# liangheming/simple_pose

Measured on AMD Instinct MI355X. Metric: images/sec fwd+decode, ResNet50-DConv 256x192 bs=128, higher is better.
Workload: dtype f32; 1 GPU; ResNet50-DConv 256x192 bs=128 per GPU, fp32 forward (NCHW in -> heat maps) + GaussTaylor decode, eval-mode BN, conditioned random weights; images_per_gpu=128, global_batch=128, parallelism=replicas x1 (no collective), ranks=1 process(es), one per GPU, launch=stream launches, tile_table=profiles/r06_dconv_f32_tiles.json, batches_in_flight=2, decode=in line, HSA_ENABLE_IPC_MODE_LEGACY=0

## Files before the change

include/simple_pose_hip.h:

```cpp
#ifndef SIMPLE_POSE_HIP_H
#define SIMPLE_POSE_HIP_H

#include <stdint.h>

#ifdef __cplusplus
extern "C" {
#endif

#define SP_OK 0
#define SP_EINVAL (-1)
#define SP_ELAUNCH (-2)

#define SP_ABI_VERSION 36

#define SP_CONV_RELU 0x1u
#define SP_CONV_OUT_NCHW 0x2u
#define SP_CONV_PIXEL_SHUFFLE 0x4u
#define SP_CONV_OUT_F32 0x10u
#define SP_CONV_BN_Y_MASK 0x20u
#define SP_CONV_BF16 0x8u
#define SP_CONV_HARDSWISH 0x40u
#define SP_CONV_OUT_SLICE 0x80u

typedef struct sp_conv_desc {
// ... 44 lines not shown
int sp_basic_block_c64(const sp_conv_desc* desc, const void* x, const void* w1_packed, const float* scale1, const float* shift1,
                       const void* w2_packed, const float* scale2, const float* shift2, void* y, void* stream);

int sp_dual_pw_bf16_ok(int64_t rows, int c_main, int c_short, int c_out);
int sp_dual_pw_f32_ok(int64_t rows, int c_main, int c_short, int c_out);
int sp_dual_pw_f32(const float* a_main, const float* w_main_packed, const float* scale_main, const float* shift_main, const float* a_short,
                   const float* w_short_packed, const float* scale_short, const float* shift_short, float* y, int64_t rows, int c_main, int c_short,
                   int c_out, int relu, void* stream);
int sp_dual_pw_bf16(const void* a_main, const void* w_main_packed, const float* scale_main, const float* shift_main, const void* a_short,
                    const void* w_short_packed, const float* scale_short, const float* shift_short, void* y, int64_t rows, int c_main, int c_short,
                    int c_out, int relu, void* stream);
int sp_pw_chain_f32_ok(int64_t rows, int c_mid, int c_out, int c_next);
int sp_pw_chain_f32(const float* t, const float* w3_packed, const float* scale3, const float* shift3, const float* residual, float* y,
                    const float* w1_packed, const float* scale1, const float* shift1, float* t_next, int64_t rows, int c_mid, int c_out, int c_next,
                    void* stream);
int sp_bottleneck_c64_ok(const sp_conv_desc* desc);
int sp_bottleneck_c64(const sp_conv_desc* desc, const void* x, const void* w1_packed, const float* scale1, const float* shift1,
                      const void* w2_packed, const float* scale2, const float* shift2, const void* w3_packed, const float* scale3,
                      const float* shift3, void* y, void* stream);

int sp_stem7_pool_ok(int batch, int h, int w);
int sp_stem7_pool(const float* x, const void* w_packed, int k_pad, const float* scale, const float* shift, void* y, int bf16,
                  int batch, int h, int w, void* stream);
int sp_stem7_pool_u8(const unsigned char* crops_bgr, const float* mean_rgb_host, const void* w_packed, int k_pad, const float* scale,
                     const float* shift, void* y, int bf16, int batch, int h, int w, void* stream);

int sp_hrnet_transition1_ok(int c_in, int h, int w);
int sp_hrnet_transition1(const void* x, int batch, int h, int w, const void* wa_packed, int k_pad, const float* scale_a, const float* shift_a,
                         const void* wb_packed, const float* scale_b, const float* shift_b, void* y_hi, void* y_lo, void* stream);
int sp_hrnet_stem_ok(int batch, int h, int w);
// ... 339 lines not shown
```

simple_pose_amd/_lib.py:

```python
from __future__ import annotations

import ctypes
import os
from ctypes import c_double, c_float, c_int, c_int32, c_int64, c_uint32, c_void_p

from .build import LIB_PATH as _DEFAULT_LIB_PATH

LIB_PATH = os.environ.get("SIMPLE_POSE_HIP_LIB", _DEFAULT_LIB_PATH)

SP_CONV_RELU = 0x1
SP_CONV_OUT_NCHW = 0x2
SP_CONV_PIXEL_SHUFFLE = 0x4
SP_CONV_BF16 = 0x8
SP_CONV_OUT_F32 = 0x10
SP_CONV_BN_Y_MASK = 0x20
SP_CONV_HARDSWISH = 0x40
SP_CONV_OUT_SLICE = 0x80
SP_LETTERBOX_FOCUS, SP_LETTERBOX_U8 = 0, 1
SP_YOLO_NMS_MAX_CANDIDATES, SP_YOLO_NMS_MAX_DET = 32768, 1024
SP_COCO_MAX_JOINTS, SP_COCO_MAX_GT_PER_IMAGE, SP_COCO_MAX_DT_PER_IMAGE, SP_COCO_MAX_DETS = 64, 128, 2048, 32
SP_COCO_DT_XY_F64, SP_COCO_DT_SCORE_F64, SP_COCO_GT_CROWD, SP_COCO_GT_IGNORE = 1, 2, 1, 2
CONV_TILES =((128, 128), (64, 128), (128, 64), (64, 64), (256, 64), (128, 32))
ABI_VERSION = 36
SP_CONV_KERNEL_IGEMM, SP_CONV_KERNEL_RING, SP_CONV_KERNEL_PW, SP_CONV_KERNEL_RING_LW, SP_CONV_KERNEL_RING_LW4 = 0, 1, 2, 3, 4
RING_LW4_TILES = ((192, 128), (128, 128), (96, 128), (256, 128), (128, 256), (96, 256), (64, 128))
RING_LW_TILES = ((256, 128), (128, 256), (256, 64), (128, 128), (192, 128))
RING_TILES = ((256, 256), (256, 128), (128, 256), (256, 64), (128, 128), (192, 128), (192, 256))


class HipLibraryError(RuntimeError):
    pass


class ConvDesc(ctypes.Structure):
    _fields_ = [(n, c_int32) for n in (
        "batch", "in_h", "in_w", "c_in", "grid_h", "grid_w", "c_out", "n_pad", "taps_h", "taps_w", "k_pad", "stride",
        "dy0", "dy_step", "dx0", "dx_step", "out_h", "out_w", "out_c", "oy_mul", "oy_add", "ox_mul", "ox_add",
# ... 122 lines not shown
    "sp_bn_fold_bwd_apply_nhwc": (c_int, [_P, c_int, _P, _P, _P, _P, _P, c_int, c_int, _P, _P, _P, c_int64, c_int64, c_int, _P, _P, _P, _P, _P, _P, c_int, _P]),
    "sp_bn_bwd_sums_from_conv": (c_int, [_P, _P, c_int, c_int, c_int, _P, _P, _P]),
    "sp_bn_bwd_sums_from_conv_pair": (c_int, [_P, _P, _P, c_int, c_int, c_int, _P, _P, _P, _P, _P]),
    "sp_u8hwc_bgr_to_nhwc": (c_int, [_P, _P, c_int, c_int, c_int, c_int, _P, _P]),
    "sp_nchw_to_nhwc4_bf16": (c_int, [_P, _P, c_int, c_int, c_int, c_int, _P]),
    "sp_conv3x3_direct_ok": (c_int, [ctypes.POINTER(ConvDesc)]),
    "sp_conv3x3_direct": (c_int, [ctypes.POINTER(ConvDesc), _P, _P, _P, _P, _P, _P, _P]),
    "sp_basic_block_c32_ok": (c_int, [ctypes.POINTER(ConvDesc)]),
    "sp_basic_block_c32": (c_int, [ctypes.POINTER(ConvDesc), _P, _P, _P, _P, _P, _P, _P, _P, _P]),
    "sp_basic_block_c64_ok": (c_int, [ctypes.POINTER(ConvDesc)]),
    "sp_basic_block_c64": (c_int, [ctypes.POINTER(ConvDesc), _P, _P, _P, _P, _P, _P, _P, _P, _P]),
    "sp_dual_pw_bf16_ok": (c_int, [c_int64, c_int, c_int, c_int]),
    "sp_dual_pw_f32_ok": (c_int, [c_int64, c_int, c_int, c_int]),
    "sp_dual_pw_f32": (c_int, [_P, _P, _P, _P, _P, _P, _P, _P, _P, c_int64, c_int, c_int, c_int, c_int, _P]),
    "sp_dual_pw_bf16": (c_int, [_P, _P, _P, _P, _P, _P, _P, _P, _P, c_int64, c_int, c_int, c_int, c_int, _P]),
    "sp_pw_chain_f32_ok": (c_int, [c_int64, c_int, c_int, c_int]),
    "sp_pw_chain_f32": (c_int, [_P, _P, _P, _P, _P, _P, _P, _P, _P, _P, c_int64, c_int, c_int, c_int, _P]),
    "sp_bottleneck_c64_ok": (c_int, [ctypes.POINTER(ConvDesc)]),
    "sp_conv2d_pw_ok": (c_int, [ctypes.POINTER(ConvDesc)]),
    "sp_hrnet_stem_ok": (c_int, [c_int, c_int, c_int]),
    "sp_hrnet_stem": (c_int, [_P, _P, c_int, _P, _P, _P, _P, _P, _P, c_int, c_int, c_int, _P]),
    "sp_hrnet_transition1_ok": (c_int, [c_int, c_int, c_int]),
    "sp_hrnet_transition1": (c_int, [_P, c_int, c_int, c_int, _P, c_int, _P, _P, _P, _P, _P, _P, _P, _P]),
    "sp_stem7_pool_ok": (c_int, [c_int, c_int, c_int]),
    "sp_stem7_pool": (c_int, [_P, _P, c_int, _P, _P, _P, c_int, c_int, c_int, c_int, _P]),
    "sp_stem7_pool_u8": (c_int, [_P, ctypes.POINTER(ctypes.c_float), _P, c_int, _P, _P, _P, c_int, c_int, c_int, c_int, _P]),
    "sp_bottleneck_c64": (c_int, [ctypes.POINTER(ConvDesc), _P, _P, _P, _P, _P, _P, _P, _P, _P, _P, _P, _P]),
    "sp_masked_mse": (c_int, [_P, _P, _P, c_int, c_int, c_int, _P, _P, _P, _P]),
    "sp_conv_packed_dims": (c_int, [c_int, c_int, c_int, ctypes.POINTER(c_int), ctypes.POINTER(c_int)]),
    "sp_pack_conv_weights": (c_int, [_P, c_int, c_int, c_int, c_int, c_int, c_int, c_int, c_int, c_int, c_int, _P, c_int, _P]),
# ... 41 lines not shown
        for name, (res, args) in SYMBOLS.items():
            fn = getattr(handle, name)
            fn.restype, fn.argtypes = res, args
        if handle.sp_abi_version() != ABI_VERSION:
            raise HipLibraryError(f"ABI mismatch: library {handle.sp_abi_version()} vs binding {ABI_VERSION}")
        _lib = handle
    return _lib


def conv_kernel_name(desc, has_residual: bool = False, variant: int = 0) -> str:
    buf = ctypes.create_string_buffer(256)
    check(lib().sp_conv2d_kernel_name(desc, int(has_residual), variant, buf, 256), "sp_conv2d_kernel_name")
    return buf.value.decode()


def check(rc: int, what: str = ""):
    if rc != 0:
        msg = lib().sp_last_error().decode("utf-8", "replace")
        raise HipLibraryError(f"{what or 'libsimple_pose_hip'} failed (code {rc}): {msg}")


def ptr(t):
    return None if t is None else t.data_ptr()


import threading

_pin = threading.local()


# ... 51 lines not shown
```

simple_pose_amd/csrc/conv_igemm.hip:

```cpp
#include "sp_common.h"
#include <stdlib.h>
#include <type_traits>

#ifdef SP_DIAG
__device__ unsigned long long sp_dbg[4096 * 4 * 12];
extern "C" int sp_debug_read(unsigned long long* dst, int n) {
    return (int)hipMemcpyFromSymbol(dst, HIP_SYMBOL(sp_dbg), sizeof(unsigned long long) * n, 0, hipMemcpyDeviceToHost);
}
extern "C" int sp_debug_clear() {
    static unsigned long long z[4096 * 4 * 12];
    return (int)hipMemcpyToSymbol(HIP_SYMBOL(sp_dbg), z, sizeof(z), 0, hipMemcpyHostToDevice);
}
#define SP_STAMP_ALWAYS(var)                                                                \
    unsigned long long var;                                                                 \
    __builtin_amdgcn_sched_barrier(0);                                                      \
    asm volatile("s_memtime %0\n\ts_waitcnt lgkmcnt(0)" : "=s"(var)::"memory");           \
    __builtin_amdgcn_sched_barrier(0);
#ifdef SP_DIAG_LIGHT
#define SP_STAMP(var) unsigned long long var = 0;
#else
#define SP_STAMP(var) SP_STAMP_ALWAYS(var)
#endif
#else
#define SP_STAMP(var)
// ... 906 lines not shown
        if ((a.flags & SP_CONV_BF16) && !(a.flags & SP_CONV_OUT_F32)) return launch_t<BM, BN, WR, WC, true, true, false, false, true>(a, phases, uniform, stream);
        if (a.flags & SP_CONV_BF16) return launch_t<BM, BN, WR, WC, true, false, false, false, true>(a, phases, uniform, stream);
        return launch_t<BM, BN, WR, WC, false, false, false, false, true>(a, phases, uniform, stream);
    }
    if (a.stats_s) {
        if (a.flags & SP_CONV_BF16) return launch_t<BM, BN, WR, WC, true, true, true>(a, phases, uniform, stream);
        return launch_t<BM, BN, WR, WC, false, false, true>(a, phases, uniform, stream);
    }
    if (a.flags & SP_CONV_BF16) {
        if (a.flags & SP_CONV_OUT_F32) return launch_t<BM, BN, WR, WC, true, false, false>(a, phases, uniform, stream);
        return launch_t<BM, BN, WR, WC, true, true, false>(a, phases, uniform, stream);
    }
    return launch_t<BM, BN, WR, WC, false, false, false>(a, phases, uniform, stream);
}

}

extern "C" int sp_conv2d_default_tile(const sp_conv_desc* d, int* tile_m, int* tile_n);
int sp_conv_ring_launch(const sp_conv_desc* d, const void* x, const void* w_packed, const float* scale, const float* shift,
                        const void* residual, void* y, void* stream);
int sp_conv_pw_launch(const sp_conv_desc* d, const void* x, const void* w_packed, const float* scale, const float* shift,
                      const void* residual, void* y, void* stream);

static int tile_rows_per_block(int, int) { return 1; }

static int g_tap_skip = -1;
static bool tap_skip_enabled() {
    if (g_tap_skip < 0) { const char* e = getenv("SP_CONV_TAP_SKIP"); g_tap_skip = (e && atoi(e) == 0) ? 0 : 1; }
    return g_tap_skip != 0;
}
// ... 292 lines not shown
        return conv_fwd_impl(&descs[0], dz, w_packed[0], nullptr, nullptr, accumulate, dx, sum_g, sum_g_xhat, stats_rows_capacity, stream, &src, &phs);
    }
    return conv_fwd_impl(&descs[0], dz, w_packed[0], nullptr, nullptr, accumulate, dx, nullptr, nullptr, 0, stream, nullptr, &phs);
}

extern "C" int sp_conv2d_dgrad_bn_bwd_stats_macc(const sp_conv_desc* d, const void* dz, const void* w_packed, const void* acc_dy, const void* acc_mask,
                                                void* dx, const void* bn_y, const void* bn_z, const float* bn_mean, const float* bn_invstd, float* sum_g,
                                                float* sum_g_xhat, const void* bn2_z, const float* bn2_mean, const float* bn2_invstd, float* sum_g_xhat2,
                                                int stats_rows_capacity, void* stream) {
    SP_REQUIRE(acc_dy && acc_mask, "sp_conv2d_dgrad_bn_bwd_stats_macc: null accumulate operand");
    SP_REQUIRE(!bn2_z || (bn2_mean && bn2_invstd && sum_g_xhat2), "sp_conv2d_dgrad_bn_bwd_stats_macc: null pointer");
    BnBwdSrc src = {bn_y, bn_z, bn_mean, bn_invstd, bn2_z, bn2_mean, bn2_invstd, sum_g_xhat2};
    src.res_mask = acc_mask;
    return conv_fwd_impl(d, dz, w_packed, nullptr, nullptr, acc_dy, dx, sum_g, sum_g_xhat, stats_rows_capacity, stream, &src);
}
```

simple_pose_amd/engine.py:

```python
from __future__ import annotations

import ctypes
import os

from dataclasses import dataclass, field
from typing import Dict, List, Optional, Tuple

import torch

from . import _lib, conv_geometry
from ._lib import ConvDesc, SP_CONV_BF16, SP_CONV_HARDSWISH, SP_CONV_OUT_NCHW, SP_CONV_OUT_SLICE, SP_CONV_PIXEL_SHUFFLE, SP_CONV_RELU
from .conv_geometry import n_pad_for, round_up as _round_up

BN_EPS = 1e-5


class HipPacker:

    @staticmethod
    def _dims(c_out: int, k: int, bf16: bool) -> Tuple[int, int]:
        n_pad, k_pad = ctypes.c_int(0), ctypes.c_int(0)
        _lib.check(_lib.lib().sp_conv_packed_dims(c_out, k, int(bf16), ctypes.byref(n_pad), ctypes.byref(k_pad)), "sp_conv_packed_dims")
        return n_pad.value, k_pad.value

# ... 174 lines not shown
                                              P(bufs[op.dst]), stream), op.name)
        elif op.kind == "bneck64":
            op.desc.batch = B
            w1, s1, h1, w3, s3, h3 = op.args
            _lib.check(lib.sp_bottleneck_c64(op.desc, P(bufs[op.src]), P(w1), P(s1), P(h1), P(op.w), P(op.scale), P(op.shift), P(w3), P(s3), P(h3),
                                             P(bufs[op.dst]), stream), op.name)
        elif op.kind == "dual1x1":
            w_s, s_s, h_s, rows_per_image, relu = op.args
            fn = lib.sp_dual_pw_bf16 if op.w.element_size() == 2 else lib.sp_dual_pw_f32
            _lib.check(fn(P(bufs[op.src]), P(op.w), P(op.scale), P(op.shift), P(bufs[op.res]), P(w_s), P(s_s), P(h_s), P(bufs[op.dst]),
                                           B * rows_per_image, 64, 64, 256, relu, stream), op.name)
        elif op.kind == "pwchain":
            w1, s1, h1, rows_per_image, c_next, _ = op.args
            _lib.check(lib.sp_pw_chain_f32(P(bufs[op.src]), P(op.w), P(op.scale), P(op.shift), P(bufs[op.res]), P(bufs[op.dst]), P(w1), P(s1), P(h1),
                                           P(bufs[op.dst2]), B * rows_per_image, 64, 256, c_next, stream), op.name)
        elif op.kind == "stem7":
            h, w, k_pad, unfused = op.args
            src = bufs[op.src]
            if src.dtype == torch.uint8:
                mean = (ctypes.c_float * 3)(0.485, 0.456, 0.406)
                _lib.check(lib.sp_stem7_pool_u8(P(src), mean, P(op.w), k_pad, P(op.scale), P(op.shift), P(bufs[op.dst]), int(self.dtype == "bf16"),
                                                B, h, w, stream), op.name)
            else:
                _lib.check(lib.sp_stem7_pool(P(src), P(op.w), k_pad, P(op.scale), P(op.shift), P(bufs[op.dst]), int(self.dtype == "bf16"),
                                             B, h, w, stream), op.name)
        elif op.kind == "htrans":
            h, w, k_pad, wb, sb, hb, _ = op.args
            _lib.check(lib.sp_hrnet_transition1(P(bufs[op.src]), B, h, w, P(op.w), k_pad, P(op.scale), P(op.shift), P(wb), P(sb), P(hb),
                                                P(bufs[op.dst]), P(bufs[op.dst2]), stream), op.name)
        elif op.kind == "hstem":
# ... 195 lines not shown
                        print(f"  {op.name:28s} {cand[0]:3d}x{cand[1]:<3d} k{cand[2]} {timed[-1][0] * 1e3:8.1f} us")
                timed.sort()
                ranked[key] = timed
                best = timed[0]
                if len(timed) > 1 and timed[1][0] < 1.08 * timed[0][0]:
                    ta, tb = [], []
                    for _ in range(rounds):
                        ta.append(time_once(op, timed[0][1], 3 * reps))
                        tb.append(time_once(op, timed[1][1], 3 * reps))
                    ma, mb = sorted(ta)[rounds // 2], sorted(tb)[rounds // 2]
                    best = (ma, timed[0][1]) if ma <= mb else (mb, timed[1][1])
                chosen[key] = best[1]
            apply(op, chosen[key])
            report[op.name] = chosen[key]
            by_key.setdefault(key, []).append(op)
        self.tuned_for_batch = B
        n_lanes = 1 + max((op.lane for op in self.ops), default=0)
        if refine is None:
            refine = self.multi_stream and n_lanes > 1
        if in_situ and not (self.multi_stream and n_lanes > 1):
            report.update(self._retime_in_situ(x, by_key, ranked, chosen, apply, verbose))
        if refine:
            report.update(self._refine_on_whole_step(x, by_key, ranked, chosen, apply, verbose))
        return report

    def _retime_in_situ(self, x, by_key, ranked, chosen, apply, verbose, top: int = 4, reps: int = 3) -> Dict[str, Tuple[int, int, int]]:
        lib = _lib.lib()
        B = x.shape[0]
        bufs = dict(self._alloc(B, x.device))
        bufs["input"] = x
# ... 60 lines not shown
            for cand in alts:
                for op in by_key[key]:
                    apply(op, cand)
                t = min(self._step_ms(x), self._step_ms(x))
                if t < base * 0.996:
                    if verbose:
                        print(f"  refine {by_key[key][0].name:28s} x{len(by_key[key])}: {chosen[key]} -> {cand}: step {base:.3f} -> {t:.3f} ms")
                    base, chosen[key] = t, cand
                else:
                    for op in by_key[key]:
                        apply(op, chosen[key])
            for op in by_key[key]:
                changed[op.name] = chosen[key]
        return changed

    def tiles(self) -> Dict[str, Tuple[int, int, int]]:
        return {op.name: ((-1, -1, 0) if op.direct else (op.desc.tile_m, op.desc.tile_n, op.desc.kernel)) for op in self.ops if op.kind == "conv"}

    def set_tiles(self, tiles: Dict[str, Tuple[int, ...]], batch: int) -> None:
        for op in self.ops:
            if op.kind == "conv" and op.name in tiles:
                t = [int(v) for v in tiles[op.name]]
                if op.desc.c_in_group:
                    if t[0] > 0 and t[1] == op.desc.c_in_group and (len(t) < 3 or t[2] == _lib.SP_CONV_KERNEL_IGEMM):
                        op.desc.tile_m = t[0]
                    continue
                op.direct = t[0] < 0
                if not op.direct:
                    op.desc.tile_m, op.desc.tile_n = t[0], t[1]
                    op.desc.kernel = t[2] if len(t) > 2 else _lib.SP_CONV_KERNEL_IGEMM
        self.tuned_for_batch = batch

    @property
    def flops_per_image(self) -> int:
        return sum(op.flops for op in self.ops)
# ... 140 lines not shown
                del table[key]
        self._hm = [None] * self.depth


class ProgramBuilder:

    def __init__(self, in_h: int, in_w: int, dtype: str = "fp32", packer=None):
        if dtype not in ("fp32", "bf16"):
            raise ValueError(dtype)
        self.packer = packer or HipPacker()
        self.fuse_blocks = False
        self.fuse_blocks64 = False
        self.fuse_bottlenecks = False
        self.fuse_tail = os.environ.get("SP_FUSE_TAIL", "1") != "0"
        self.fuse_chain = os.environ.get("SP_FUSE_CHAIN", "1") != "0"
        self.fuse_stem = True
        self.fuse_terms = True
        self.fuse_transition = True
        self.p = Program(dtype=dtype)
        self.bf16 = dtype == "bf16"
        self.cpad = 8 if self.bf16 else 4
        self.p.shapes["input"] = (in_h, in_w, 3)
        self._n = 0
        self.lane = 0

    def _add(self, op: Op) -> None:
        op.lane = self.lane
        self.p.ops.append(op)

    def _fresh(self, stem: str) -> str:
# ... 128 lines not shown
    def dual_pointwise_tail(self, main: str, w3, s3, h3, short: str, wd, sd_, hd, name: str) -> Optional[str]:
        h, w, c = self.p.shapes[main]
        hs, ws_, cs = self.p.shapes[short]
        ok = _lib.lib().sp_dual_pw_bf16_ok if self.bf16 else _lib.lib().sp_dual_pw_f32_ok
        if not (self.fuse_tail and (h, w) == (hs, ws_) and c == 64 and cs == 64 and tuple(w3.shape) == (256, 64, 1, 1)
                and tuple(wd.shape) == (256, 64, 1, 1) and ok(h * w, 64, 64, 256)):
            return None
        p3, pd = self.packer.conv(w3, bf16=self.bf16)[0], self.packer.conv(wd, bf16=self.bf16)[0]
        if tuple(p3.shape) != (256, 64) or tuple(pd.shape) != (256, 64):
            return None
        dst = self._fresh(name)
        self.p.shapes[dst] = (h, w, 256)
        self._add(Op("dual1x1", main, dst, res=short, w=p3, scale=s3, shift=h3, args=(pd, sd_, hd, h * w, 1), name=name, flops=2 * h * w * 2 * 64 * 256))
        return dst

    def deconv_k4s2p1(self, src: str, weight: torch.Tensor, *, scale=None, shift=None, relu: bool = False,
                      name: str = "deconv") -> str:
        h, w, c = self.p.shapes[src]
        I, O = weight.shape[:2]
        assert I == c
        packed, n_pad = self.packer.deconv(weight, bf16=self.bf16)
        d = conv_geometry.deconv_k4s2p1_fwd(h, w, I, O, n_pad, (SP_CONV_RELU if relu else 0) | (SP_CONV_BF16 if self.bf16 else 0))
        dst = self._fresh(name)
        self.p.shapes[dst] = (2 * h, 2 * w, O)
        self._add(Op("conv", src, dst, desc=d, w=packed, scale=scale, shift=shift,
                             name=name, flops=2 * h * w * I * O * 16))
        return dst

    def pixel_shuffle(self, src: str) -> str:
        h, w, c = self.p.shapes[src]
# ... 66 lines not shown
        y = b.bottleneck_c64(x, sd[p + ".conv1.weight"], s1, h1, sd[p + ".conv2.weight"], s2, h2, sd[p + ".conv3.weight"], s3, h3, name=p)
        if y is not None:
            return y
    s1, h1 = _bn(b, sd, p + ".bn1")
    t = b.conv(x, sd[p + ".conv1.weight"], scale=s1, shift=h1, relu=True, name=p + ".conv1")
    s2, h2 = _bn(b, sd, p + ".bn2")
    w2 = sd[p + ".conv2.weight"]
    t = b.conv(t, w2, stride=stride, pad=1, scale=s2, shift=h2, relu=True, name=p + ".conv2", groups=w2.shape[0] // w2.shape[1])
    idn = x
    if (p + ".downsample.0.weight") in sd and stride == 1 and (p + ".se.fc.0.weight") not in sd and w2.shape[0] == w2.shape[1]:
        sdn, hdn = _bn(b, sd, p + ".downsample.1")
        s3, h3 = _bn(b, sd, p + ".bn3")
        y = b.dual_pointwise_tail(t, sd[p + ".conv3.weight"], s3, h3, x, sd[p + ".downsample.0.weight"], sdn, hdn, name=p + ".conv3+downsample")
        if y is not None:
            return y
    if (p + ".downsample.0.weight") in sd:
        sdn, hdn = _bn(b, sd, p + ".downsample.1")
        idn = b.conv(x, sd[p + ".downsample.0.weight"], stride=stride, scale=sdn, shift=hdn, name=p + ".downsample")
    s3, h3 = _bn(b, sd, p + ".bn3")
    if (p + ".se.fc.0.weight") in sd:
        z = b.conv(t, sd[p + ".conv3.weight"], scale=s3, shift=h3, name=p + ".conv3")
        g = b.gap(z)
        g = b.conv(g, sd[p + ".se.fc.0.weight"], shift=b.packer.bias(sd[p + ".se.fc.0.bias"]), relu=True, name=p + ".se.fc.0")
        g = b.conv(g, sd[p + ".se.fc.2.weight"], shift=b.packer.bias(sd[p + ".se.fc.2.bias"]), name=p + ".se.fc.2")
        return b.se_gate(z, g, idn)
    return b.conv(t, sd[p + ".conv3.weight"], scale=s3, shift=h3, relu=True, res=idn, name=p + ".conv3")


def _res_basic_block(b: ProgramBuilder, sd, x: str, p: str, stride: int) -> str:
    s1, h1 = _bn(b, sd, p + ".bn1")
# ... 34 lines not shown
                  dc.c_out in (64, 128) and tuple(a.w.shape) == (256, 64) and tuple(c.w.shape) == (dc.c_out, 256) and
                  _lib.lib().sp_pw_chain_f32_ok(da.grid_h * da.grid_w, 64, 256, dc.c_out))
        if ok:
            out.append(Op("pwchain", a.src, a.dst, res=a.res, dst2=c.dst, w=a.w, scale=a.scale, shift=a.shift,
                          args=(c.w, c.scale, c.shift, da.grid_h * da.grid_w, dc.c_out, (a, c)), name=a.name + "+" + c.name, flops=a.flops + c.flops,
                          lane=a.lane))
            i += 2
        else:
            out.append(a)
            i += 1
    b.p.ops[:] = out


def resnet_program(sd: Dict[str, torch.Tensor], head: str, in_h: int = 256, in_w: int = 192,
                   blocks=(3, 4, 6, 3), dtype: str = "fp32", packer=None, fuse_bottlenecks: bool = False, fuse_stem: bool = True,
                   fuse_chain: bool = False) -> Program:
    b = ProgramBuilder(in_h, in_w, dtype, packer)
    b.fuse_bottlenecks = fuse_bottlenecks
    b.fuse_tail = fuse_bottlenecks and b.fuse_tail
    b.fuse_stem = fuse_stem
    s, h = _bn(b, sd, "bn1")
    x = b.stem_pool("input", sd["conv1.weight"], s, h, name="conv1")
    basic = "layer1.0.conv3.weight" not in sd
    for li, n in enumerate(blocks, start=1):
        for bi in range(n):
            x = (_res_basic_block if basic else _bottleneck)(b, sd, x, f"layer{li}.{bi}", 2 if (bi == 0 and li > 1) else 1)
    if fuse_chain and not basic:
        _fuse_pw_chains(b, sd)
    J = sd["final_layer.weight"].shape[0]
    if head == "dconv":
        for idx in (0, 3, 6):
            s, h = _bn(b, sd, f"deconv_layers.{idx + 1}")
            x = b.deconv_k4s2p1(x, sd[f"deconv_layers.{idx}.weight"], scale=s, shift=h, relu=True,
                                name=f"deconv_layers.{idx}")
        b.conv(x, sd["final_layer.weight"], shift=b.packer.bias(sd["final_layer.bias"]), out_nchw=True,
# ... 272 lines not shown
```

simple_pose_amd/nets/_resnet_base.py:

```python
from __future__ import annotations

from typing import Optional

import torch
from torch import nn

from .. import engine
from .._lib import HipLibraryError, require_cuda_f32
from ..metrics.flip import COCO_JOINT_PAIRS, merge_flipped, mirror_input, pairs_to_perm


class _Bottleneck(nn.Module):
    expansion = 4

    def __init__(self, inplanes: int, planes: int, stride: int, with_downsample: bool, with_se: bool = False, width: int = 0, groups: int = 1):
        super().__init__()
        width = width or planes
        self.conv1 = nn.Conv2d(inplanes, width, 1, bias=False)
        self.bn1 = nn.BatchNorm2d(width)
        self.conv2 = nn.Conv2d(width, width, 3, stride=stride, padding=1, groups=groups, bias=False)
        self.bn2 = nn.BatchNorm2d(width)
        self.conv3 = nn.Conv2d(width, planes * 4, 1, bias=False)
        self.bn3 = nn.BatchNorm2d(planes * 4)
        if with_downsample:
# ... 69 lines not shown
        for m in self.modules():
            if isinstance(m, (nn.Conv2d, nn.ConvTranspose2d)):
                nn.init.normal_(m.weight, std=0.001)
                if m.bias is not None:
                    nn.init.constant_(m.bias, 0)
            elif isinstance(m, nn.BatchNorm2d):
                nn.init.constant_(m.weight, 1)
                nn.init.constant_(m.bias, 0)

    def _build_head(self, inplanes: int, num_classes: int):
        raise NotImplementedError

    fuse_bottlenecks = True
    fuse_stem = True
    fuse_chain = True

    def _tensors_key(self, x):
        sd = self.state_dict(keep_vars=True)
        return (tuple(x.shape[2:]), str(x.device), self.compute_dtype, self.fuse_bottlenecks, self.fuse_stem, self.fuse_chain) + tuple((v.data_ptr(), v._version) for v in sd.values())

    def hip_program(self, x: torch.Tensor) -> engine.Program:
        key = self._tensors_key(x)
        if self._program is None or key != self._program_key:
            sd = {k: v.detach() for k, v in self.state_dict(keep_vars=True).items()}
            for k, v in sd.items():
                if v.device != x.device:
                    raise HipLibraryError(f"parameter {k} is on {v.device} but the input is on {x.device}; call .to(device)")
            self._program = engine.resnet_program(sd, self.HEAD, in_h=x.shape[2], in_w=x.shape[3], blocks=self.BLOCKS,
                                                   dtype=self.compute_dtype, fuse_bottlenecks=self.fuse_bottlenecks, fuse_stem=self.fuse_stem,
                                                   fuse_chain=self.fuse_chain)
            self._program_key = key
        return self._program

    def forward(self, x: torch.Tensor) -> torch.Tensor:
        x = require_cuda_f32(x, "input")
        if x.dim() != 4 or x.shape[1] != 3 or x.shape[2] % 32 or x.shape[3] % 32:
            raise ValueError(f"expected [B,3,H,W] with H,W multiples of 32, got {tuple(x.shape)}")
        if self.training:
            return self._forward_train(x)
        prog = self.hip_program(x)
        if self.autotune and x.shape[0] >= 16 and x.shape[0] >= 4 * prog.tuned_for_batch:
            prog.autotune(x)
        return prog.run(x)

    def _forward_train(self, x: torch.Tensor) -> torch.Tensor:
# ... 73 lines not shown
```

Before: 11870 images/s.

## Fuse bottleneck conv3 and downsample 1x1 convs into one dual implicit-GEMM kernel

```diff
diff --git a/include/simple_pose_hip.h b/include/simple_pose_hip.h
--- a/include/simple_pose_hip.h
+++ b/include/simple_pose_hip.h
@@ -82,6 +82,11 @@
 int sp_pw_chain_f32(const float* t, const float* w3_packed, const float* scale3, const float* shift3, const float* residual, float* y,
                     const float* w1_packed, const float* scale1, const float* shift1, float* t_next, int64_t rows, int c_mid, int c_out, int c_next,
                     void* stream);
+int sp_conv2d_dual_f32_ok(const sp_conv_desc* d_main, const sp_conv_desc* d_short);
+int sp_conv2d_dual_f32(const sp_conv_desc* d_main, const void* t, const void* w3_packed, const float* scale3, const float* shift3,
+                       const sp_conv_desc* d_short, const void* x, const void* wd_packed, const float* scale_d, const float* shift_d, void* y,
+                       void* stream);
+int sp_conv2d_dual_kernel_name(const sp_conv_desc* d_main, const sp_conv_desc* d_short, char* buf, int cap);
 int sp_bottleneck_c64_ok(const sp_conv_desc* desc);
 int sp_bottleneck_c64(const sp_conv_desc* desc, const void* x, const void* w1_packed, const float* scale1, const float* shift1,
                       const void* w2_packed, const float* scale2, const float* shift2, const void* w3_packed, const float* scale3,
diff --git a/simple_pose_amd/_lib.py b/simple_pose_amd/_lib.py
--- a/simple_pose_amd/_lib.py
+++ b/simple_pose_amd/_lib.py
@@ -21,6 +21,7 @@
 SP_COCO_MAX_JOINTS, SP_COCO_MAX_GT_PER_IMAGE, SP_COCO_MAX_DT_PER_IMAGE, SP_COCO_MAX_DETS = 64, 128, 2048, 32
 SP_COCO_DT_XY_F64, SP_COCO_DT_SCORE_F64, SP_COCO_GT_CROWD, SP_COCO_GT_IGNORE = 1, 2, 1, 2
 CONV_TILES =((128, 128), (64, 128), (128, 64), (64, 64), (256, 64), (128, 32))
+DUAL_TILES = ((128, 128), (128, 64), (64, 128), (64, 64))
 ABI_VERSION = 36
 SP_CONV_KERNEL_IGEMM, SP_CONV_KERNEL_RING, SP_CONV_KERNEL_PW, SP_CONV_KERNEL_RING_LW, SP_CONV_KERNEL_RING_LW4 = 0, 1, 2, 3, 4
 RING_LW4_TILES = ((192, 128), (128, 128), (96, 128), (256, 128), (128, 256), (96, 256), (64, 128))
@@ -173,6 +174,9 @@
     "sp_dual_pw_f32_ok": (c_int, [c_int64, c_int, c_int, c_int]),
     "sp_dual_pw_f32": (c_int, [_P, _P, _P, _P, _P, _P, _P, _P, _P, c_int64, c_int, c_int, c_int, c_int, _P]),
     "sp_dual_pw_bf16": (c_int, [_P, _P, _P, _P, _P, _P, _P, _P, _P, c_int64, c_int, c_int, c_int, c_int, _P]),
+    "sp_conv2d_dual_f32_ok": (c_int, [ctypes.POINTER(ConvDesc), ctypes.POINTER(ConvDesc)]),
+    "sp_conv2d_dual_f32": (c_int, [ctypes.POINTER(ConvDesc), _P, _P, _P, _P, ctypes.POINTER(ConvDesc), _P, _P, _P, _P, _P, _P]),
+    "sp_conv2d_dual_kernel_name": (c_int, [ctypes.POINTER(ConvDesc), ctypes.POINTER(ConvDesc), ctypes.c_char_p, c_int]),
     "sp_pw_chain_f32_ok": (c_int, [c_int64, c_int, c_int, c_int]),
     "sp_pw_chain_f32": (c_int, [_P, _P, _P, _P, _P, _P, _P, _P, _P, _P, c_int64, c_int, c_int, c_int, _P]),
     "sp_bottleneck_c64_ok": (c_int, [ctypes.POINTER(ConvDesc)]),
@@ -244,6 +248,12 @@
     return buf.value.decode()
 
 
+def dual_kernel_name(d_main, d_short) -> str:
+    buf = ctypes.create_string_buffer(256)
+    check(lib().sp_conv2d_dual_kernel_name(d_main, d_short, buf, 256), "sp_conv2d_dual_kernel_name")
+    return buf.value.decode()
+
+
 def check(rc: int, what: str = ""):
     if rc != 0:
         msg = lib().sp_last_error().decode("utf-8", "replace")
diff --git a/simple_pose_amd/csrc/conv_igemm.hip b/simple_pose_amd/csrc/conv_igemm.hip
--- a/simple_pose_amd/csrc/conv_igemm.hip
+++ b/simple_pose_amd/csrc/conv_igemm.hip
@@ -944,6 +944,271 @@
     return launch_t<BM, BN, WR, WC, false, false, false>(a, phases, uniform, stream);
 }
 
+struct DualArgs {
+    const void* x;
+    const void* t;
+    const void* wd;
+    const void* w3;
+    const float* scale_d;
+    const float* shift_d;
+    const float* scale3;
+    const float* shift3;
+    void* y;
+    int M;
+    int in_h, in_w, stride;
+    int grid_h, grid_w;
+    int c_short, c_mid, c_out, n_pad;
+    int relu;
+    int tiles_m, tiles_n;
+    int x_bytes, t_bytes, wd_bytes, w3_bytes, y_bytes;
+};
+
+template <int BM, int BN, int WR, int WC>
+__global__ __launch_bounds__(256, 2) void conv_igemm_dual_kernel(const DualArgs p) {
+    static_assert(WR * WC == 4, "4 waves per workgroup");
+    constexpr int WM = BM / WR, WN = BN / WC;
+    constexpr int TM = WM / 32, TN = WN / 32;
+    constexpr int A_CH = BM / 32, B_CH = BN / 32;
+    static_assert(TM >= 1 && TN >= 1, "wave tile must hold at least one 32x32 MFMA tile");
+
+    extern __shared__ __attribute__((aligned(16))) float smem[];
+    float* As = smem;
+    float* Bs = smem + 2 * BM * BK;
+    int* rowtab = reinterpret_cast<int*>(smem + 2 * (BM + BN) * BK);
+
+    const int tid = threadIdx.x;
+    const int lane = tid & 63;
+    const int wave = __builtin_amdgcn_readfirstlane(tid >> 6);
+    const int wr = wave / WC, wc = wave % WC;
+
+    const int nwg = p.tiles_m * p.tiles_n;
+    int t;
+    {
+        const int orig = blockIdx.x;
+        const int xcd = orig & 7, q = nwg >> 3, r = nwg & 7;
+        t = (xcd < r ? xcd * (q + 1) : r * (q + 1) + (xcd - r) * q) + (orig >> 3);
+    }
+    const int tn = t % p.tiles_n, tm = t / p.tiles_n;
+    const int m0 = tm * BM, n0 = tn * BN;
+
+    constexpr unsigned OOB = 0x80000000u;
+    if (tid < BM) {
+        const int m = m0 + tid;
+        int4 e;
+        if (m < p.M) {
+            const int gw = p.grid_w, ghw = p.grid_h * gw;
+            const int b = m / ghw;
+            const int rem = m - b * ghw;
+            const int gy = rem / gw, gx = rem - gy * gw;
+            e.x = ((b * p.in_h + gy * p.stride) * p.in_w + gx * p.stride) * p.c_short * 4;
+            e.y = 1;
+            e.z = m * p.c_mid * 4;
+            e.w = m * p.c_out;
+        } else {
+            e.x = (int)OOB; e.y = 0; e.z = (int)OOB; e.w = -1;
+        }
+        reinterpret_cast<int4*>(rowtab)[tid] = e;
+    }
+    __syncthreads();
+
+    const __amdgpu_buffer_rsrc_t xr = __builtin_amdgcn_make_buffer_rsrc(const_cast<void*>(p.x), (short)0, p.x_bytes, 0x00020000);
+    const __amdgpu_buffer_rsrc_t tr_ = __builtin_amdgcn_make_buffer_rsrc(const_cast<void*>(p.t), (short)0, p.t_bytes, 0x00020000);
+    const __amdgpu_buffer_rsrc_t wdr = __builtin_amdgcn_make_buffer_rsrc(const_cast<void*>(p.wd), (short)0, p.wd_bytes, 0x00020000);
+    const __amdgpu_buffer_rsrc_t w3r = __builtin_amdgcn_make_buffer_rsrc(const_cast<void*>(p.w3), (short)0, p.w3_bytes, 0x00020000);
+    const int kc = tid & 7;
+    const int srow = tid >> 3;
+    unsigned a_off[2][A_CH];
+#pragma unroll
+    for (int i = 0; i < A_CH; ++i) {
+        const int4 e = reinterpret_cast<const int4*>(rowtab)[srow + 32 * i];
+        a_off[0][i] = e.y ? (unsigned)(e.x + kc * 16) : OOB;
+        a_off[1][i] = e.y ? (unsigned)(e.z + kc * 16) : OOB;
+    }
+    const unsigned b_voff[2] = {(unsigned)((srow * p.c_short + kc * 4) * 4), (unsigned)((srow * p.c_mid + kc * 4) * 4)};
+    const unsigned b_row[2] = {(unsigned)(32 * p.c_short * 4), (unsigned)(32 * p.c_mid * 4)};
+    const unsigned b_soff0[2] = {(unsigned)n0 * p.c_short * 4, (unsigned)n0 * p.c_mid * 4};
+
+    u32x4 sa[A_CH], sb[B_CH];
+    using P0 = std::integral_constant<int, 0>;
+    using P1 = std::integral_constant<int, 1>;
+    auto load_a = [&](int i, auto pass_tag, int k0) {
+        constexpr int PASS = decltype(pass_tag)::value;
+        if constexpr (PASS == 0) sa[i] = __builtin_amdgcn_raw_buffer_load_b128(xr, a_off[0][i] + (unsigned)(k0 * 4), 0, 0);
+        else sa[i] = __builtin_amdgcn_raw_buffer_load_b128(tr_, a_off[1][i] + (unsigned)(k0 * 4), 0, 0);
+    };
+    auto load_b = [&](int i, auto pass_tag, int k0) {
+        constexpr int PASS = decltype(pass_tag)::value;
+        if constexpr (PASS == 0) sb[i] = __builtin_amdgcn_raw_buffer_load_b128(wdr, b_voff[0] + (unsigned)i * b_row[0], b_soff0[0] + (unsigned)(k0 * 4), 0);
+        else sb[i] = __builtin_amdgcn_raw_buffer_load_b128(w3r, b_voff[1] + (unsigned)i * b_row[1], b_soff0[1] + (unsigned)(k0 * 4), 0);
+    };
+    auto store_piece = [&](int buf, int o) {
+        if (o < A_CH) *reinterpret_cast<u32x4*>(As + buf * BM * BK + swz(srow + 32 * o, kc)) = sa[o];
+        else *reinterpret_cast<u32x4*>(Bs + buf * BN * BK + swz(srow + 32 * (o - A_CH), kc)) = sb[o - A_CH];
+    };
+
+    f32x16 acc[TM][TN], z[TM][TN];
+#pragma unroll
+    for (int i = 0; i < TM; ++i)
+#pragma unroll
+        for (int n = 0; n < TN; ++n)
+#pragma unroll
+            for (int r = 0; r < 16; ++r) acc[i][n][r] = 0.f;
+
+    const int fr = lane & 31, fh = lane >> 5;
+    const int nk1 = p.c_short / BK, nk2 = p.c_mid / BK;
+
+    f32x4 fa[2][TM], fb[2][TN];
+    auto read_frags = [&](const float* a, const float* b, int j, int slot) {
+#pragma unroll
+        for (int i = 0; i < TM; ++i) fa[slot][i] = *reinterpret_cast<const f32x4*>(a + swz(i * 32 + fr, 2 * j + fh));
+#pragma unroll
+        for (int n = 0; n < TN; ++n) fb[slot][n] = *reinterpret_cast<const f32x4*>(b + swz(n * 32 + fr, 2 * j + fh));
+    };
+    constexpr int NM = 4 * TM * TN;
+    constexpr int NOPS = A_CH + B_CH;
+    auto mfma_q = [&](int slot, int q) {
+        const int s = q / (TM * TN), i = (q / TN) % TM, n = q % TN;
+        acc[i][n] = __builtin_amdgcn_mfma_f32_32x32x2f32(fa[slot][i][s], fb[slot][n][s], acc[i][n], 0, 0, 0);
+    };
+#define SP_SB() __builtin_amdgcn_sched_barrier(0)
+
+#pragma unroll
+    for (int i = 0; i < A_CH; ++i) load_a(i, P0{}, 0);
+#pragma unroll
+    for (int i = 0; i < B_CH; ++i) load_b(i, P0{}, 0);
+#pragma unroll
+    for (int o = 0; o < NOPS; ++o) store_piece(0, o);
+    __syncthreads();
+    read_frags(As + (wr * WM) * BK, Bs + (wc * WN) * BK, 0, 0);
+
+    auto k_tile = [&](int g, auto more_tag, auto next_tag, int next_k0) {
+        constexpr bool MORE = decltype(more_tag)::value;
+        const int cur = g & 1;
+        const float* a = As + cur * BM * BK + (wr * WM) * BK;
+        const float* b = Bs + cur * BN * BK + (wc * WN) * BK;
+        const float* an = As + (cur ^ 1) * BM * BK + (wr * WM) * BK;
+        const float* bn = Bs + (cur ^ 1) * BN * BK + (wc * WN) * BK;
+        read_frags(a, b, 1, 1);
+        SP_SB();
+#pragma unroll
+        for (int q = 0; q < NM; ++q) {
+            mfma_q(0, q);
+            if (MORE) {
+#pragma unroll
+                for (int o = (q * NOPS) / NM; o < ((q + 1) * NOPS) / NM; ++o) {
+                    if (o < A_CH) load_a(o, next_tag, next_k0); else load_b(o - A_CH, next_tag, next_k0);
+                }
+            }
+            SP_SB();
+        }
+        read_frags(a, b, 2, 0);
+#pragma unroll
+        for (int q = 0; q < NM; ++q) mfma_q(1, q);
+        SP_SB();
+        read_frags(a, b, 3, 1);
+#pragma unroll
+        for (int q = 0; q < NM; ++q) mfma_q(0, q);
+        SP_SB();
+        constexpr int H3 = NM / 2;
+#pragma unroll
+        for (int q = 0; q < H3; ++q) {
+            mfma_q(1, q);
+            if (MORE) {
+#pragma unroll
+                for (int o = (q * NOPS) / H3; o < ((q + 1) * NOPS) / H3; ++o) store_piece(cur ^ 1, o);
+            }
+            SP_SB();
+        }
+        if (MORE) {
+            __syncthreads();
+            read_frags(an, bn, 0, 0);
+            SP_SB();
+        }
+#pragma unroll
+        for (int q = NM / 2; q < NM; ++q) mfma_q(1, q);
+        SP_SB();
+    };
+
+    float scd[TN], shd[TN], sc3[TN], sh3[TN];
+#pragma unroll
+    for (int n = 0; n < TN; ++n) {
+        const int col = n0 + wc * WN + n * 32 + fr;
+        const bool col_ok = col < p.c_out;
+        scd[n] = (col_ok && p.scale_d) ? p.scale_d[col] : 1.f;
+        shd[n] = (col_ok && p.shift_d) ? p.shift_d[col] : 0.f;
+    }
+
+    int g = 0;
+    for (int kt = 0; kt + 1 < nk1; ++kt, ++g) k_tile(g, std::true_type{}, P0{}, (kt + 1) * BK);
+    k_tile(g++, std::true_type{}, P1{}, 0);
+#pragma unroll
+    for (int i = 0; i < TM; ++i)
+#pragma unroll
+        for (int n = 0; n < TN; ++n)
+#pragma unroll
+            for (int r = 0; r < 16; ++r) {
+                z[i][n][r] = acc[i][n][r] * scd[n] + shd[n];
+                acc[i][n][r] = 0.f;
+            }
+#pragma unroll
+    for (int n = 0; n < TN; ++n) {
+        const int col = n0 + wc * WN + n * 32 + fr;
+        const bool col_ok = col < p.c_out;
+        sc3[n] = (col_ok && p.scale3) ? p.scale3[col] : 1.f;
+        sh3[n] = (col_ok && p.shift3) ? p.shift3[col] : 0.f;
+    }
+    SP_SB();
+    for (int kt = 0; kt + 1 < nk2; ++kt, ++g) k_tile(g, std::true_type{}, P1{}, (kt + 1) * BK);
+    k_tile(g, std::false_type{}, P1{}, 0);
+    __syncthreads();
+#undef SP_SB
+
+    static_assert(BM * BN <= 2 * (BM + BN) * BK, "transpose area must fit in the staging buffers");
+    const bool relu = p.relu != 0;
+    const __amdgpu_buffer_rsrc_t yr = __builtin_amdgcn_make_buffer_rsrc(p.y, (short)0, p.y_bytes, 0x00020000);
+    float* tr = smem + wave * (WM * WN);
+#pragma unroll
+    for (int i = 0; i < TM; ++i)
+#pragma unroll
+        for (int n = 0; n < TN; ++n)
+#pragma unroll
+            for (int r = 0; r < 16; ++r) {
+                float v = acc[i][n][r];
+                v = v * sc3[n] + sh3[n];
+                v += z[i][n][r];
+                if (relu) v = v > 0.f ? v : 0.f;
+                tr[(i * 32 + (r & 3) + 8 * (r >> 2) + 4 * fh) * WN + n * 32 + fr] = v;
+            }
+    constexpr int CPR = WN / 4;
+    constexpr int RPI = 64 / CPR;
+    constexpr int NIT = WM / RPI;
+    const int chunk = lane % CPR, rsub = lane / CPR;
+    const int col = n0 + wc * WN + chunk * 4;
+    const bool col_ok = col < p.c_out;
+#pragma unroll
+    for (int it = 0; it < NIT; ++it) {
+        const int ro = rowtab[(wr * WM + it * RPI + rsub) * 4 + 3];
+        const unsigned off = (col_ok && ro >= 0) ? (unsigned)((ro + col) * 4) : OOB;
+        const u32x4 o = *reinterpret_cast<const u32x4*>(tr + (it * RPI + rsub) * WN + chunk * 4);
+        __builtin_amdgcn_raw_buffer_store_b128(o, yr, off, 0, 0);
+    }
+}
+
+template <int BM, int BN, int WR, int WC>
+int launch_dual(const DualArgs& a, hipStream_t stream) {
+    if (sp_name_query_active()) {
+        sp_name_query_set("conv_igemm_dual_kernel<%d, %d, %d, %d>", BM, BN, WR, WC);
+        return SP_OK;
+    }
+    DualArgs p = a;
+    p.tiles_m = (a.M + BM - 1) / BM;
+    p.tiles_n = a.n_pad / BN;
+    const size_t lds = (size_t)2 * (BM + BN) * BK * sizeof(float) + (size_t)BM * 4 * sizeof(int);
+    if (sp_reserve_lds<&conv_igemm_dual_kernel<BM, BN, WR, WC>>((int)lds, "conv_igemm_dual")) return SP_ELAUNCH;
+    hipLaunchKernelGGL((conv_igemm_dual_kernel<BM, BN, WR, WC>), dim3(p.tiles_m * p.tiles_n, 1, 1), dim3(256, 1, 1), lds, stream, p);
+    return sp_check_launch("conv_igemm_dual_kernel");
+}
+
 }
 
 extern "C" int sp_conv2d_default_tile(const sp_conv_desc* d, int* tile_m, int* tile_n);
@@ -1266,3 +1531,92 @@
     src.res_mask = acc_mask;
     return conv_fwd_impl(d, dz, w_packed, nullptr, nullptr, acc_dy, dx, sum_g, sum_g_xhat, stats_rows_capacity, stream, &src);
 }
+
+static const char* dual_refusal(const sp_conv_desc* m, const sp_conv_desc* s) {
+    if (!m || !s) return "null descriptor";
+    const unsigned barred = SP_CONV_BF16 | SP_CONV_OUT_F32 | SP_CONV_OUT_NCHW | SP_CONV_PIXEL_SHUFFLE | SP_CONV_OUT_SLICE | SP_CONV_HARDSWISH | SP_CONV_BN_Y_MASK;
+    if ((m->flags | s->flags) & SP_CONV_BF16) return "fp32 only (a descriptor carries SP_CONV_BF16)";
+    if ((m->flags | s->flags) & SP_CONV_OUT_NCHW) return "needs an NHWC store (a descriptor carries SP_CONV_OUT_NCHW)";
+    if ((m->flags | s->flags) & SP_CONV_PIXEL_SHUFFLE) return "no pixel shuffle";
+    if ((m->flags | s->flags) & barred) return "no slice, hardswish or mask epilogue";
+    if ((m->flags & ~(barred | SP_CONV_RELU)) || (s->flags & ~barred)) return "unknown flag bits (the shortcut descriptor carries no ReLU)";
+    for (const sp_conv_desc* d : {m, s}) {
+        if (d->c_in_group != 0) return "grouped convolutions are not taken";
+        if (d->taps_h != 1 || d->taps_w != 1 || d->phases_y != 1 || d->phases_x != 1 || d->dy0 != 0 || d->dx0 != 0) return "both convolutions must be 1x1, one phase, no padding";
+        if (d->c_in <= 0 || d->c_in % BK != 0 || d->k_pad != d->c_in) return "c_in must fill whole K tiles (c_in % 32 == 0, k_pad == c_in)";
+        if (d->kernel != SP_CONV_KERNEL_IGEMM) return "the implicit-GEMM kernel only";
+        if (d->batch <= 0 || d->grid_h <= 0 || d->grid_w <= 0 || d->in_h <= 0 || d->in_w <= 0) return "non-positive dimension";
+        if (d->out_h != d->grid_h || d->out_w != d->grid_w || d->oy_mul != 1 || d->ox_mul != 1 || d->oy_add != 0 || d->ox_add != 0 || d->out_c != d->c_out)
+            return "the output grid must be the output tensor";
+    }
+    if (m->batch != s->batch) return "the descriptors differ in batch";
+    if (m->grid_h != s->grid_h || m->grid_w != s->grid_w) return "the descriptors differ in output grid";
+    if (m->c_out != s->c_out || m->n_pad != s->n_pad) return "the descriptors differ in c_out / n_pad";
+    if (m->tile_m != s->tile_m || m->tile_n != s->tile_n) return "the descriptors differ in tile";
+    if (m->c_out <= 0 || m->c_out % 4 != 0 || m->n_pad % 32 != 0 || m->n_pad < m->c_out) return "c_out must be a multiple of 4 and n_pad a multiple of 32 >= c_out";
+    if (m->stride != 1 || m->stride_x > 1 || m->in_h != m->grid_h || m->in_w != m->grid_w) return "the main convolution must be stride 1 on the output grid";
+    if ((s->stride != 1 && s->stride != 2) || (s->stride_x != 0 && s->stride_x != s->stride)) return "the shortcut must be stride 1 or 2";
+    if ((s->grid_h - 1) * s->stride >= s->in_h || (s->grid_w - 1) * s->stride >= s->in_w) return "the shortcut's output grid leaves its input";
+    const long long M = (long long)m->batch * m->grid_h * m->grid_w;
+    const long long lim = 1ll << 29;
+    if (M >= lim || M * m->c_in >= lim || M * m->c_out >= lim || (long long)s->batch * s->in_h * s->in_w * s->c_in >= lim ||
+        (long long)m->n_pad * m->c_in >= lim || (long long)s->n_pad * s->c_in >= lim)
+        return "tensor too large (each operand must stay below 2 GiB for 32-bit buffer offsets)";
+    int bm = m->tile_m, bn = m->tile_n;
+    if (bm == 0 && bn == 0) sp_conv2d_default_tile(s, &bm, &bn);
+    if (!((bm == 128 || bm == 64) && (bn == 128 || bn == 64))) return "unsupported tile (supported: 128x128 128x64 64x128 64x64)";
+    if (m->n_pad % bn != 0) return "tile_n must divide n_pad";
+    return nullptr;
+}
+
+extern "C" int sp_conv2d_dual_f32_ok(const sp_conv_desc* d_main, const sp_conv_desc* d_short) {
+    return dual_refusal(d_main, d_short) == nullptr ? 1 : 0;
+}
+
+static int conv_dual_impl(const sp_conv_desc* dm, const void* t, const void* w3, const float* scale3, const float* shift3, const sp_conv_desc* ds,
+                          const void* x, const void* wd, const float* scale_d, const float* shift_d, void* y, void* stream) {
+    SP_REQUIRE(dm && ds && t && w3 && x && wd && y, "sp_conv2d_dual_f32: null pointer");
+    const char* why = dual_refusal(dm, ds);
+    SP_REQUIRE(!why, "sp_conv2d_dual_f32: %s", why);
+    SP_REQUIRE(y != t && y != x, "sp_conv2d_dual_f32: y must not alias an input");
+    const long long M = (long long)dm->batch * dm->grid_h * dm->grid_w;
+    DualArgs a;
+    a.x = x; a.t = t; a.wd = wd; a.w3 = w3; a.scale_d = scale_d; a.shift_d = shift_d; a.scale3 = scale3; a.shift3 = shift3; a.y = y;
+    a.M = (int)M;
+    a.in_h = ds->in_h; a.in_w = ds->in_w; a.stride = ds->stride;
+    a.grid_h = dm->grid_h; a.grid_w = dm->grid_w;
+    a.c_short = ds->c_in; a.c_mid = dm->c_in; a.c_out = dm->c_out; a.n_pad = dm->n_pad;
+    a.relu = (dm->flags & SP_CONV_RELU) ? 1 : 0;
+    a.tiles_m = a.tiles_n = 0;
+    a.x_bytes = (int)((long long)ds->batch * ds->in_h * ds->in_w * ds->c_in * 4);
+    a.t_bytes = (int)(M * dm->c_in * 4);
+    a.wd_bytes = (int)((long long)ds->n_pad * ds->c_in * 4);
+    a.w3_bytes = (int)((long long)dm->n_pad * dm->c_in * 4);
+    a.y_bytes = (int)(M * dm->c_out * 4);
+    int bm = dm->tile_m, bn = dm->tile_n;
+    if (bm == 0 && bn == 0) sp_conv2d_default_tile(ds, &bm, &bn);
+    hipStream_t s = (hipStream_t)stream;
+    if (bm == 128 && bn == 128) return launch_dual<128, 128, 2, 2>(a, s);
+    if (bm == 128 && bn == 64) return launch_dual<128, 64, 2, 2>(a, s);
+    if (bm == 64 && bn == 128) return launch_dual<64, 128, 2, 2>(a, s);
+    return launch_dual<64, 64, 2, 2>(a, s);
+}
+
+extern "C" int sp_conv2d_dual_f32(const sp_conv_desc* d_main, const void* t, const void* w3_packed, const float* scale3, const float* shift3,
+                                  const sp_conv_desc* d_short, const void* x, const void* wd_packed, const float* scale_d, const float* shift_d,
+                                  void* y, void* stream) {
+    return conv_dual_impl(d_main, t, w3_packed, scale3, shift3, d_short, x, wd_packed, scale_d, shift_d, y, stream);
+}
+
+extern "C" int sp_conv2d_dual_kernel_name(const sp_conv_desc* d_main, const sp_conv_desc* d_short, char* buf, int cap) {
+    SP_REQUIRE(d_main && d_short && buf && cap > 0, "sp_conv2d_dual_kernel_name: null pointer");
+    void* const dummy = reinterpret_cast<void*>(16);
+    void* const dummy2 = reinterpret_cast<void*>(32);
+    void* const dummy3 = reinterpret_cast<void*>(48);
+    sp_name_query_begin();
+    const int rc = conv_dual_impl(d_main, dummy, dummy, nullptr, nullptr, d_short, dummy2, dummy, nullptr, nullptr, dummy3, nullptr);
+    const char* name = sp_name_query_end();
+    if (rc != SP_OK) return rc;
+    snprintf(buf, (size_t)cap, "%s", name);
+    return SP_OK;
+}
diff --git a/simple_pose_amd/engine.py b/simple_pose_amd/engine.py
--- a/simple_pose_amd/engine.py
+++ b/simple_pose_amd/engine.py
@@ -212,6 +212,11 @@
             w1, s1, h1, rows_per_image, c_next, _ = op.args
             _lib.check(lib.sp_pw_chain_f32(P(bufs[op.src]), P(op.w), P(op.scale), P(op.shift), P(bufs[op.res]), P(bufs[op.dst]), P(w1), P(s1), P(h1),
                                            P(bufs[op.dst2]), B * rows_per_image, 64, 256, c_next, stream), op.name)
+        elif op.kind == "dualconv":
+            d_short, w_s, s_s, h_s, _ = op.args
+            op.desc.batch = d_short.batch = B
+            _lib.check(lib.sp_conv2d_dual_f32(op.desc, P(bufs[op.src]), P(op.w), P(op.scale), P(op.shift), d_short, P(bufs[op.res]), P(w_s), P(s_s), P(h_s),
+                                              P(bufs[op.dst]), stream), op.name)
         elif op.kind == "stem7":
             h, w, k_pad, unfused = op.args
             src = bufs[op.src]
@@ -437,6 +442,30 @@
             apply(op, chosen[key])
             report[op.name] = chosen[key]
             by_key.setdefault(key, []).append(op)
+        for op in self.ops:
+            if op.kind != "dualconv":
+                continue
+            timed = []
+            for bm, bn in _lib.DUAL_TILES:
+                if op.desc.n_pad % bn:
+                    continue
+                self._set_dual_tile(op, bm, bn)
+                self._launch(lib, op, bufs, B, stream)
+                ts = []
+                for _ in range(rounds):
+                    e0, e1 = torch.cuda.Event(enable_timing=True), torch.cuda.Event(enable_timing=True)
+                    e0.record()
+                    for _ in range(reps):
+                        self._launch(lib, op, bufs, B, stream)
+                    e1.record()
+                    e1.synchronize()
+                    ts.append(e0.elapsed_time(e1) / reps)
+                timed.append((sorted(ts)[len(ts) // 2], (bm, bn, _lib.SP_CONV_KERNEL_IGEMM)))
+                if verbose:
+                    print(f"  {op.name:28s} {bm:3d}x{bn:<3d} dual {timed[-1][0] * 1e3:8.1f} us")
+            best = min(timed)[1]
+            self._set_dual_tile(op, best[0], best[1])
+            report[op.name] = best
         self.tuned_for_batch = B
         n_lanes = 1 + max((op.lane for op in self.ops), default=0)
         if refine is None:
@@ -527,11 +556,22 @@
                 changed[op.name] = chosen[key]
         return changed
 
+    @staticmethod
+    def _set_dual_tile(op: Op, bm: int, bn: int) -> None:
+        for d in (op.desc, op.args[0]):
+            d.tile_m, d.tile_n, d.kernel = bm, bn, _lib.SP_CONV_KERNEL_IGEMM
+
     def tiles(self) -> Dict[str, Tuple[int, int, int]]:
-        return {op.name: ((-1, -1, 0) if op.direct else (op.desc.tile_m, op.desc.tile_n, op.desc.kernel)) for op in self.ops if op.kind == "conv"}
+        return {op.name: ((-1, -1, 0) if op.direct else (op.desc.tile_m, op.desc.tile_n, op.desc.kernel)) for op in self.ops if op.kind in ("conv", "dualconv")}
 
     def set_tiles(self, tiles: Dict[str, Tuple[int, ...]], batch: int) -> None:
         for op in self.ops:
+            if op.kind == "dualconv":
+                t = tiles.get(op.name) or tiles.get(op.name.split(".conv3+")[0] + ".downsample")
+                if t is not None and (int(t[0]), int(t[1])) in _lib.DUAL_TILES and (len(t) < 3 or int(t[2]) == _lib.SP_CONV_KERNEL_IGEMM) and \
+                        op.desc.n_pad % int(t[1]) == 0:
+                    self._set_dual_tile(op, int(t[0]), int(t[1]))
+                continue
             if op.kind == "conv" and op.name in tiles:
                 t = [int(v) for v in tiles[op.name]]
                 if op.desc.c_in_group:
@@ -702,6 +742,7 @@
         self.fuse_bottlenecks = False
         self.fuse_tail = os.environ.get("SP_FUSE_TAIL", "1") != "0"
         self.fuse_chain = os.environ.get("SP_FUSE_CHAIN", "1") != "0"
+        self.fuse_dual = False
         self.fuse_stem = True
         self.fuse_terms = True
         self.fuse_transition = True
@@ -860,6 +901,18 @@
         self._add(Op("dual1x1", main, dst, res=short, w=p3, scale=s3, shift=h3, args=(pd, sd_, hd, h * w, 1), name=name, flops=2 * h * w * 2 * 64 * 256))
         return dst
 
+    def dual_conv_tail(self, main: str, w3, s3, h3, short: str, wd, sd_, hd, stride: int, block: str) -> str:
+        first = len(self.p.ops)
+        idn = self.conv(short, wd, stride=stride, scale=sd_, shift=hd, name=block + ".downsample")
+        y = self.conv(main, w3, scale=s3, shift=h3, relu=True, res=idn, name=block + ".conv3")
+        ds, c3 = self.p.ops[first:]
+        if self.bf16 or ds.direct or c3.direct or not _lib.lib().sp_conv2d_dual_f32_ok(c3.desc, ds.desc):
+            return y
+        del self.p.ops[first:]
+        self._add(Op("dualconv", main, y, res=short, desc=c3.desc, w=c3.w, scale=s3, shift=h3, args=(ds.desc, ds.w, sd_, hd, (ds, c3)),
+                     name=block + ".conv3+downsample", flops=ds.flops + c3.flops))
+        return y
+
     def deconv_k4s2p1(self, src: str, weight: torch.Tensor, *, scale=None, shift=None, relu: bool = False,
                       name: str = "deconv") -> str:
         h, w, c = self.p.shapes[src]
@@ -956,6 +1009,11 @@
         y = b.dual_pointwise_tail(t, sd[p + ".conv3.weight"], s3, h3, x, sd[p + ".downsample.0.weight"], sdn, hdn, name=p + ".conv3+downsample")
         if y is not None:
             return y
+    if (b.fuse_dual and not b.bf16 and (p + ".downsample.0.weight") in sd and (p + ".se.fc.0.weight") not in sd and w2.shape[0] == w2.shape[1] and
+            not (stride == 1 and tuple(sd[p + ".conv3.weight"].shape) == (256, 64, 1, 1) and tuple(sd[p + ".downsample.0.weight"].shape) == (256, 64, 1, 1))):
+        sdn, hdn = _bn(b, sd, p + ".downsample.1")
+        s3, h3 = _bn(b, sd, p + ".bn3")
+        return b.dual_conv_tail(t, sd[p + ".conv3.weight"], s3, h3, x, sd[p + ".downsample.0.weight"], sdn, hdn, stride, p)
     if (p + ".downsample.0.weight") in sd:
         sdn, hdn = _bn(b, sd, p + ".downsample.1")
         idn = b.conv(x, sd[p + ".downsample.0.weight"], stride=stride, scale=sdn, shift=hdn, name=p + ".downsample")
@@ -1020,11 +1078,12 @@
 
 def resnet_program(sd: Dict[str, torch.Tensor], head: str, in_h: int = 256, in_w: int = 192,
                    blocks=(3, 4, 6, 3), dtype: str = "fp32", packer=None, fuse_bottlenecks: bool = False, fuse_stem: bool = True,
-                   fuse_chain: bool = False) -> Program:
+                   fuse_chain: bool = False, fuse_dual: bool = False) -> Program:
     b = ProgramBuilder(in_h, in_w, dtype, packer)
     b.fuse_bottlenecks = fuse_bottlenecks
     b.fuse_tail = fuse_bottlenecks and b.fuse_tail
     b.fuse_stem = fuse_stem
+    b.fuse_dual = fuse_dual and os.environ.get("SP_FUSE_DUAL", "1") != "0"
     s, h = _bn(b, sd, "bn1")
     x = b.stem_pool("input", sd["conv1.weight"], s, h, name="conv1")
     basic = "layer1.0.conv3.weight" not in sd
diff --git a/simple_pose_amd/nets/_resnet_base.py b/simple_pose_amd/nets/_resnet_base.py
--- a/simple_pose_amd/nets/_resnet_base.py
+++ b/simple_pose_amd/nets/_resnet_base.py
@@ -107,10 +107,11 @@
     fuse_bottlenecks = True
     fuse_stem = True
     fuse_chain = True
+    fuse_dual = True
 
     def _tensors_key(self, x):
         sd = self.state_dict(keep_vars=True)
-        return (tuple(x.shape[2:]), str(x.device), self.compute_dtype, self.fuse_bottlenecks, self.fuse_stem, self.fuse_chain) + tuple((v.data_ptr(), v._version) for v in sd.values())
+        return (tuple(x.shape[2:]), str(x.device), self.compute_dtype, self.fuse_bottlenecks, self.fuse_stem, self.fuse_chain, self.fuse_dual) + tuple((v.data_ptr(), v._version) for v in sd.values())
 
     def hip_program(self, x: torch.Tensor) -> engine.Program:
         key = self._tensors_key(x)
@@ -121,7 +122,7 @@
                     raise HipLibraryError(f"parameter {k} is on {v.device} but the input is on {x.device}; call .to(device)")
             self._program = engine.resnet_program(sd, self.HEAD, in_h=x.shape[2], in_w=x.shape[3], blocks=self.BLOCKS,
                                                    dtype=self.compute_dtype, fuse_bottlenecks=self.fuse_bottlenecks, fuse_stem=self.fuse_stem,
-                                                   fuse_chain=self.fuse_chain)
+                                                   fuse_chain=self.fuse_chain, fuse_dual=self.fuse_dual)
             self._program_key = key
         return self._program
 
```

New measurement: 11970 images/s, median of 6. No clear change (+0.8%).
